# Giovannibriglia/ContinuousBayesianNetwork

Hardware: AMD Instinct MI355X
Metric: marginal queries/sec + achieved HBM GB/s, 20-node d=32 DAG, 65k-batch VE (higher is better)
Workload: dtype f32; 1 GPU; chain20_d32: BayesianNetwork.infer target X19, evidence on the other 19 nodes, N_max=32; queries_per_gpu=65536, global_batch=65536, parallelism=query-shard x1

## Files before the change

continuousbayesiannetwork_amd/csrc/cbn_infer.hip:

```cpp

#include <hip/hip_runtime.h>

#include <algorithm>
#include <cstdarg>
#include <cstdint>
#include <cstdio>
#include <cstdlib>
#include <cstring>
#include <string>
#include <type_traits>
#include <vector>

#include <unistd.h>

#include "cbn_internal.h"

using namespace cbn;

namespace {
thread_local std::string g_err;
}

namespace {
const bool g_diag = [] {
// ... 109 lines not shown
__device__ unsigned g_clock_n = 0;
#define CBN_STAMP_INIT                                                                        \
    const unsigned long long _t0 = __builtin_amdgcn_s_memrealtime();                          \
    const unsigned long long _m0 = __builtin_amdgcn_s_memtime();                              \
    (void)_m0;                                                                                \
    unsigned long long* const _stp = g_stamps;                                                \
    if (_stp && (threadIdx.x & 63) == 0)                                                      \
        _stp[((size_t)blockIdx.x * (blockDim.x / 64) + threadIdx.x / 64) * 12] = _t0
#define CBN_STAMP(k)                                                                          \
    do {                                                                                      \
        __builtin_amdgcn_sched_barrier(0);                                                    \
        unsigned long long _t = __builtin_amdgcn_s_memrealtime();    \
        if (_stp && (threadIdx.x & 63) == 0)                                                  \
            _stp[((size_t)blockIdx.x * (blockDim.x / 64) + threadIdx.x / 64) * 12 + (k)] = _t; \
        __builtin_amdgcn_sched_barrier(0);                                                    \
    } while (0)
#define CBN_CLOCK_END                                                                         \
    do {                                                                                      \
        unsigned long long* const _ck = g_clock;                                              \
        if (_ck && blockIdx.x == 0 && threadIdx.x == 0) {                                     \
            const unsigned long long _m1 = __builtin_amdgcn_s_memtime();                      \
            const unsigned long long _r1 = __builtin_amdgcn_s_memrealtime();                  \
            const unsigned _i = g_clock_n;                                                    \
            if (_i < kClockRing) {                                                            \
                _ck[4 * _i] = _m0;                                                            \
                _ck[4 * _i + 1] = _t0;                                                        \
                _ck[4 * _i + 2] = _m1;                                                        \
                _ck[4 * _i + 3] = _r1;                                                        \
            }                                                                                 \
            g_clock_n = _i + 1;                                                               \
        }                                                                                     \
    } while (0)
#else
#define CBN_STAMP_INIT do {} while (0)
#define CBN_STAMP(k) do {} while (0)
#define CBN_CLOCK_END do {} while (0)
#endif

#ifdef CBN_CHECKED
__device__ unsigned* g_dbg = nullptr;
#define CBN_OK_OR(cond, code) ((cond) ? true : (g_dbg ? (atomicOr(g_dbg, 1u << (code)), atomicAdd(g_dbg + 1 + (code), 1u), false) : false))
#else
#define CBN_OK_OR(cond, code) true
#endif

typedef __attribute__((address_space(3))) void lds_void_t;
typedef const __attribute__((address_space(1))) float gfloat_t;

__device__ __forceinline__ float gload(const float* p, long long i) {
    return ((gfloat_t*)p)[i];
}
typedef const __attribute__((address_space(1))) void gbl_void_t;
typedef const __attribute__((address_space(4))) int cint_t;

typedef unsigned u32x4_t __attribute__((ext_vector_type(4)));
__device__ __forceinline__ __amdgpu_buffer_rsrc_t rows_rsrc(float* base, long long bytes) {
    return __builtin_amdgcn_make_buffer_rsrc(base, 0, (int)(bytes < 0x7fffffff ? bytes : 0x7fffffff), 0x00020000);
}
__device__ __forceinline__ void store_wt(__amdgpu_buffer_rsrc_t r, int off, float4 v) {
    u32x4_t x = {__float_as_uint(v.x), __float_as_uint(v.y), __float_as_uint(v.z), __float_as_uint(v.w)};
#ifndef CBN_STORE_AUX
#define CBN_STORE_AUX 16
#endif
    __builtin_amdgcn_raw_buffer_store_b128(x, r, off, 0, CBN_STORE_AUX);
}

__device__ __forceinline__ int4 sload_int4(const void* p) {
    const cint_t* q = reinterpret_cast<const cint_t*>(reinterpret_cast<uintptr_t>(p));
    return make_int4(q[0], q[1], q[2], q[3]);
}

__device__ __forceinline__ void lds_dma_copy(const float* __restrict__ g, float4* lds, int n4,
                                             int nw = kQueryThreads / kWave) {
    const int lane = threadIdx.x & (kWave - 1);
    const int wave = __builtin_amdgcn_readfirstlane(threadIdx.x / kWave);
    const int nchunk = (n4 + kWave - 1) / kWave;
    for (int c0 = wave; c0 < nchunk; c0 += nw) {
        const int c = (c0 + (int)blockIdx.x) % nchunk;
        const int i = c * kWave + lane;
        if (i < n4 && CBN_OK_OR(i >= 0, 0))
            __builtin_amdgcn_global_load_lds((gbl_void_t*)(g + (size_t)i * 4), (lds_void_t*)(lds + c * kWave), 16,
                                             0, 0);
    }
}

__global__ void k_cpd_scatter(const int32_t* __restrict__ cell, const float* __restrict__ prob,
                              long long n_rows, float* __restrict__ cpd) {
    for (long long r = blockIdx.x * (long long)blockDim.x + threadIdx.x; r < n_rows;
         r += (long long)gridDim.x * blockDim.x)
        cpd[cell[r]] = prob[r];
}

__global__ void k_cpd_normalize(float* __restrict__ cpd, long long n_pcells, int card) {
    for (long long c = blockIdx.x * (long long)blockDim.x + threadIdx.x; c < n_pcells;
         c += (long long)gridDim.x * blockDim.x) {
        float* row = cpd + c * card;
        double s = 0.0;
        for (int v = 0; v < card; ++v) s += (double)row[v];
        const float den = (float)s + 1e-10f;
        for (int v = 0; v < card; ++v) row[v] = row[v] / den;
    }
}

__global__ void k_cpd_eval(const float* __restrict__ cpd, int n_cols, ColPtrs cols,
                           const float* __restrict__ pts, long long n_pts, float* __restrict__ out) {
    for (long long i = blockIdx.x * (long long)blockDim.x + threadIdx.x; i < n_pts;
         i += (long long)gridDim.x * blockDim.x) {
        long long off = 0;
        bool ok = true;
        for (int c = 0; c < n_cols; ++c) {
            const int idx = bsearch_eq(cols.dom[c], cols.card[c], pts[i * n_cols + c]);
            ok &= idx >= 0;
            off += (long long)(idx < 0 ? 0 : idx) * cols.stride[c];
        }
        out[i] = ok ? cpd[off] : 0.f;
    }
}

__device__ double entry_partial(const DevFactor& d, int entry, int N, int c0, int c1, int cs) {
    if (d.kind == CBN_FACTOR_SCALAR) {
        double s = 0.0;
        for (int j = c0; j < c1; j += cs) {
            const int ni = d.node_sample_idx[j];
            s += ni >= 0 ? (double)d.cpd[ni] : 0.0;
        }
        return s;
    }
    const int row = entry / N;
    const int j = entry - row * N;
    const int ni = d.node_sample_idx[j];
    if (ni < 0) return 0.0;
    int base = ni;
    int r = row;
    for (int p = d.n_parents - 1; p >= 0; --p) {
        if (d.ev_slot[p] >= 0) {
            const int card = d.parent_card[p];
            const int q = r / card;
            base += (r - q * card) * d.cpd_stride[p];
            r = q;
        }
    }
    double s = 0.0;
    for (int c = c0; c < c1; c += cs) {
        int off = base;
        int cc = c;
        bool ok = true;
        for (int p = d.n_parents - 1; p >= 0; --p) {
            if (d.ev_slot[p] < 0) {
                const int q = cc / N;
                const int pi = d.parent_sample_idx[p * N + (cc - q * N)];
                cc = q;
                ok &= pi >= 0;
                off += (pi < 0 ? 0 : pi) * d.cpd_stride[p];
            }
        }
        s += ok ? (double)d.cpd[off] : 0.0;
    }
    return s;
}

__device__ __forceinline__ double wave_sum_d(double v) {
#pragma unroll
    for (int o = 32; o > 0; o >>= 1) v += __shfl_xor(v, o, kWave);
    return v;
}

// ... 1157 lines not shown
        }
        if (valid) {
            if (MODE == kModeFused && !first) fq = q;
            if (MODE == kModeWrite) {
                float* o = out + q * N;
#pragma unroll
                for (int v = 0; v < VPL; ++v)
                    *reinterpret_cast<float4*>(o + col[v]) = make_float4(
                        acc[4 * v] / maxv, acc[4 * v + 1] / maxv, acc[4 * v + 2] / maxv, acc[4 * v + 3] / maxv);
            } else if (MODE == kModeRaw) {
                float* o = out + q * N;
#pragma unroll
                for (int v = 0; v < VPL; ++v)
                    *reinterpret_cast<float4*>(o + col[v]) =
                        make_float4(acc[4 * v], acc[4 * v + 1], acc[4 * v + 2], acc[4 * v + 3]);
#pragma unroll
                for (int i = 0; i < NV; ++i) lmax = fmaxf(lmax, acc[i]);
            } else {
#pragma unroll
                for (int i = 0; i < NV; ++i) lmax = fmaxf(lmax, acc[i]);
            }
        }
        __builtin_amdgcn_s_waitcnt(0xC07F);
        __builtin_amdgcn_wave_barrier();
        if (first) CBN_STAMP(6);
        first = false;
    }
    CBN_STAMP(7);
    if (MODE == kModeMax || MODE == kModeRaw) {
        lmax = wave_max(lmax);
        if (lane == 0) wmax[wid] = lmax;
        __syncthreads();
        if (tid == 0) {
            float m = 0.f;
            for (int i = 0; i < nthr / kWave; ++i) m = fmaxf(m, wmax[i]);
            max_out[blockIdx.x] = __float_as_uint(m);
        }
        if (blockIdx.x == 0)
            for (int i = (int)gridDim.x + tid; i < n_max; i += nthr) max_out[i] = 0u;
    }
    if (MODE == kModeFused) {
        lmax = wave_max(lmax);
        if (lane == 0) wmax[wid] = lmax;
        __syncthreads();
        if (wid == 0) {
            const int nw = nthr / kWave;
            const unsigned gm = slot_barrier_max(sync, epoch, wave_max(lane < nw ? wmax[lane] : 0.f));
            if (lane == 0) {
                wmax[0] = __uint_as_float(gm);
                if (blockIdx.x == 0 && max_out) *max_out = gm;
            }
        }
        CBN_STAMP(8);
        __syncthreads();
        CBN_STAMP(9);
        maxv = wmax[0];
        if (fq0 >= 0) {
            float* o = out + fq0 * N;
#pragma unroll
            for (int v = 0; v < VPL; ++v)
                *reinterpret_cast<float4*>(o + col[v]) = make_float4(
                    acc0[4 * v] / maxv, acc0[4 * v + 1] / maxv, acc0[4 * v + 2] / maxv, acc0[4 * v + 3] / maxv);
        }
        if (fq >= 0) {
            float* o = out + fq * N;
#pragma unroll
            for (int v = 0; v < VPL; ++v)
                *reinterpret_cast<float4*>(o + col[v]) = make_float4(
                    acc[4 * v] / maxv, acc[4 * v + 1] / maxv, acc[4 * v + 2] / maxv, acc[4 * v + 3] / maxv);
        }
        CBN_STAMP(10);
    }
}

constexpr int kSR = 256;
constexpr int kSQ = 128;
constexpr int kSU = 4;
#ifndef CBN_DMA_WAVES
#define CBN_DMA_WAVES 4
#endif
constexpr int kDmaW = CBN_DMA_WAVES;
constexpr int kEvW = kQueryThreads / kWave - kDmaW;
constexpr int kSUp = (64 + kEvW - 1) / kEvW;

struct FoldJob {
    float* rows;
    const unsigned* words;
    long long n4;
    long long chunk;
    int n_words;
};
constexpr int kFoldK = 2;
constexpr int kFoldW = 4;

template <int MODE>
__global__ void __launch_bounds__(kQueryThreads)
k_query_staged(const float* __restrict__ gimage, int image_floats, int rec_off, int nf, int zero_off, long long Q,
               long long per, unsigned* __restrict__ sync, unsigned epoch, const unsigned* __restrict__ max_in,
               int n_max, unsigned* __restrict__ max_out, float* __restrict__ out, FoldJob fold,
               FPtrsT<kFastPtrsSmall> fp) {
    CBN_STAMP_INIT;
    constexpr int N = 32;
    extern __shared__ __attribute__((aligned(16))) float4 smem4[];
    float* simg = reinterpret_cast<float*>(smem4);
    const int T = (nf + 2) >> 1;
    const int S = (T + 1) >> 1;
    const int nsl = 4 * (S + 1);
    int* offs = reinterpret_cast<int*>(simg + image_floats);
    float* wmax = reinterpret_cast<float*>(offs + 2 * kSR * nsl);
    const int tid = threadIdx.x;
    const int lane = tid & (kWave - 1);
    const int wid = __builtin_amdgcn_readfirstlane(tid / kWave);
    const long long q0 = (long long)blockIdx.x * per;
    const long long q1 = q0 + per < Q ? q0 + per : Q;
    const int nunits = nf * (kSR / kSQ);
    const FastRec* grec = reinterpret_cast<const FastRec*>(gimage + rec_off);
    const int one_off = zero_off + 64;

    float x[kSUp][2] = {};
    auto stage_load = [&](long long qr, auto ksu, int gw, int GW) {
        constexpr int KSU = decltype(ksu)::value;
        uintptr_t pk[KSU];
#pragma unroll
        for (int k = 0; k < KSU; ++k) {
            const int u = gw + k * GW;
            pk[k] = reinterpret_cast<uintptr_t>(fp.p[((u / (kSR / kSQ)) & 31) * kFastObs]);
        }
#pragma unroll
        for (int k = 0; k < KSU; ++k) {
            const int u = gw + k * GW;
            if (u < nunits) {
                const float* col = reinterpret_cast<const float*>(pk[k] & ~(kTagMore | kTagNone));
#pragma unroll
                for (int h = 0; h < 2; ++h) {
                    const long long q = qr + (u % (kSR / kSQ)) * kSQ + h * kWave + lane;
                    x[k][h] = gload(col, (pk[k] & kTagNone) ? 0 : (q < q1 ? q : q0));
                }
            }
        }
    };
    auto stage_store = [&](long long qr, int buf, auto ksu, int gw, int GW) {
        constexpr int KSU = decltype(ksu)::value;
        int* ob = offs + buf * kSR * nsl;
        int4 rk[KSU];
#pragma unroll
        for (int k = 0; k < KSU; ++k) {
            const int u = gw + k * GW;
            rk[k] = sload_int4(grec + (u < nunits ? u / (kSR / kSQ) : 0));
        }
#pragma unroll
        for (int k = 0; k < KSU; ++k) {
            const int u = gw + k * GW;
            if (u < nunits) {
                const int f = u / (kSR / kSQ);
                const int n_obs = rk[k].y, c0 = rk[k].z;
                const int zoff = zero_off + (f & 1) * 32;
#pragma unroll
                for (int h = 0; h < 2; ++h) {
                    const int ql = (u % (kSR / kSQ)) * kSQ + h * kWave + lane;
                    int o;
                    if (n_obs == 1 && (c0 & kDenseBit)) {
                        const int card = c0 & (kDenseBit - 1);
                        const float xv = x[k][h];
                        const int i = (int)xv;
                        o = (xv >= 0.f && xv < (float)card && (float)i == xv) ? rk[k].x + i * 64 : zoff;
                    } else if (n_obs == 0) {
                        o = rk[k].x;
                    } else {
                        const FastRec& r = grec[f];
                        float xs[kFastObs];
                        xs[0] = x[k][h];
                        if (n_obs > 1) {
                            const long long q = qr + ql;
#pragma unroll
                            for (int p = 1; p < kFastObs; ++p)
                                if (p < n_obs) xs[p] = gload(fp.p[f * kFastObs + p], q < q1 ? q : q0);
                        }
                        int row = 0;
                        bool ok = true;
#pragma unroll
                        for (int p = 0; p < kFastObs; ++p) {
                            if (p < n_obs) {
                                const int card = r.card[p] & (kDenseBit - 1);
                                const float xv = xs[p];
                                int i;
                                if (r.card[p] & kDenseBit) {
                                    i = (int)xv;
                                    i = (xv >= 0.f && xv < (float)card && (float)i == xv) ? i : -1;
                                } else {
                                    i = bsearch_eq(gimage + r.dom_off[p], card, xv);
                                }
                                ok &= i >= 0;
                                row = row * card + (i < 0 ? 0 : i);
                            }
                        }
                        o = ok ? r.table_off + row * 64 : zoff;
                    }
                    ob[ql * nsl + f + ((ql >> 1) & 1)] = o;
                }
            }
        }
    };

    if (tid < kSR) {
        const int d = (tid >> 1) & 1;
        for (int j = 0; j < nsl; ++j) {
            const int f = j - d;
            if (f < 0 || f >= nf) {
                const int o = one_off + (f & 1) * 32;
                offs[tid * nsl + j] = o;
                offs[kSR * nsl + tid * nsl + j] = o;
            }
        }
    }
    long long qr = q0;
    const bool dma_wave = wid < kDmaW;
    if (!dma_wave) {
#ifndef CBN_ABL_NOSTAGE
        if (qr < q1) stage_load(qr, std::integral_constant<int, kSUp>{}, wid - kDmaW, kEvW);
#endif
    } else {
#ifndef CBN_ABL_NODMA
        lds_dma_copy(gimage, smem4, image_floats / 4, kDmaW);
#endif
    }
    CBN_STAMP(1);
    if (!dma_wave && qr < q1)
        stage_store(qr, 0, std::integral_constant<int, kSUp>{}, wid - kDmaW, kEvW);
    CBN_STAMP(2);
    __syncthreads();
    CBN_STAMP(3);
    float4 fv[kFoldK];
    unsigned fw[kFoldW];
    const long long fb = (long long)blockIdx.x * fold.chunk;
    const long long fe = fb + fold.chunk < fold.n4 ? fb + fold.chunk : fold.n4;
    if (MODE == kModeRaw && fold.rows) {
        const float4* r4 = reinterpret_cast<const float4*>(fold.rows);
#pragma unroll
        for (int k = 0; k < kFoldK; ++k) {
            const long long i = fb + tid + k * kQueryThreads;
            fv[k] = i < fe ? r4[i] : make_float4(0.f, 0.f, 0.f, 0.f);
        }
#pragma unroll
        for (int k = 0; k < kFoldW; ++k) {
            const int w = lane + k * kWave;
            fw[k] = w < fold.n_words ? fold.words[w] : 0u;
        }
    }

    const int qi = lane >> 2;
    const int l = lane & 3;
    const int h0 = qi & 1;
    const int clo = (l + 4 * h0) * 4, chi = (l + 4 * (h0 ^ 1)) * 4;
    float lmax = 0.f;
    float maxv = 1.f;
    if (MODE == kModeWrite) {
        unsigned m = 0;
        for (int i = lane; i < n_max; i += kWave) m = max(m, max_in[i]);
        m = wave_max_u(m);
        maxv = __uint_as_float(m);
        if (max_out && blockIdx.x == 0 && tid == 0) *max_out = m;
    }
    float acc[8];
    long long fq = -1;
    int buf = 0;
    const bool wt_raw = MODE == kModeRaw && fold.rows != nullptr;
    const __amdgpu_buffer_rsrc_t orsrc =
        rows_rsrc((MODE == kModeFused || wt_raw) ? out + q0 * N : nullptr,
                  (MODE == kModeFused || wt_raw) ? (q1 - q0) * (long long)(N * 4) : 0);
    for (; qr < q1; qr += kSR, buf ^= 1) {
        const long long qn = qr + kSR;
        if (MODE != kModeFused && qn < q1) stage_load(qn, std::integral_constant<int, kSU>{}, wid, kQueryThreads / kWave);
        const int ql = wid * 16 + qi;
        const long long q = qr + ql;
        const int* my = offs + buf * kSR * nsl + ql * nsl;
#pragma unroll
        for (int i = 0; i < 8; ++i) acc[i] = 1.f;
        auto mul_step = [&](const float4& r0, const float4& r1, const float4& r2, const float4& r3) {
            acc[0] *= r0.x; acc[1] *= r0.y; acc[2] *= r0.z; acc[3] *= r0.w;
            acc[4] *= r1.x; acc[5] *= r1.y; acc[6] *= r1.z; acc[7] *= r1.w;
            acc[0] *= r2.x; acc[1] *= r2.y; acc[2] *= r2.z; acc[3] *= r2.w;
            acc[4] *= r3.x; acc[5] *= r3.y; acc[6] *= r3.z; acc[7] *= r3.w;
        };
        auto load_step = [&](int oa, int ob, float4& r0, float4& r1, float4& r2, float4& r3) {
            r0 = *reinterpret_cast<const float4*>(simg + oa + clo);
            r1 = *reinterpret_cast<const float4*>(simg + oa + chi);
            r2 = *reinterpret_cast<const float4*>(simg + ob + clo);
            r3 = *reinterpret_cast<const float4*>(simg + ob + chi);
        };
        typedef float vf4 __attribute__((ext_vector_type(4)));
        typedef const volatile __attribute__((address_space(3))) vf4 lds_vf4;
        auto vld = [&](int o) {
            const vf4 v = *(lds_vf4*)(simg + o);
            return make_float4(v.x, v.y, v.z, v.w);
        };
        auto vload_step = [&](int oa, int ob, float4& r0, float4& r1, float4& r2, float4& r3) {
            r0 = vld(oa + clo);
            r1 = vld(oa + chi);
            r2 = vld(ob + clo);
            r3 = vld(ob + chi);
        };
        float4 A0, A1, A2, A3, B0, B1, B2, B3;
        int4 on = *reinterpret_cast<const int4*>(my);
        vload_step(on.x, on.y, A0, A1, A2, A3);
        vload_step(on.z, on.w, B0, B1, B2, B3);
        {
            typedef int vi4 __attribute__((ext_vector_type(4)));
            typedef const volatile __attribute__((address_space(3))) vi4 lds_vi4;
            const vi4 v = *(lds_vi4*)(my + 4);
            on = make_int4(v.x, v.y, v.z, v.w);
        }
        CBN_STAMP(4);
#ifdef CBN_ABL_NOPROD
        mul_step(A0, A1, A2, A3);
#else
#pragma unroll 2
        for (int sp = 0; sp < S; ++sp) {
            mul_step(A0, A1, A2, A3);
            load_step(on.x, on.y, A0, A1, A2, A3);
            mul_step(B0, B1, B2, B3);
            load_step(on.z, on.w, B0, B1, B2, B3);
            on = *reinterpret_cast<const int4*>(my + 4 * min(sp + 2, S));
        }
#endif
        CBN_STAMP(5);
        if (q < q1) {
            if (MODE == kModeFused) fq = q;
            if (MODE == kModeRaw && wt_raw) {
                const int ob = (int)(q - q0) * (N * 4);
                store_wt(orsrc, ob + clo * 4, make_float4(acc[0], acc[1], acc[2], acc[3]));
                store_wt(orsrc, ob + chi * 4, make_float4(acc[4], acc[5], acc[6], acc[7]));
            } else if (MODE == kModeWrite || MODE == kModeRaw) {
                const float dv = MODE == kModeWrite ? maxv : 1.f;
                float* o = out + q * N;
                *reinterpret_cast<float4*>(o + clo) = MODE == kModeWrite
                    ? make_float4(acc[0] / dv, acc[1] / dv, acc[2] / dv, acc[3] / dv)
                    : make_float4(acc[0], acc[1], acc[2], acc[3]);
                *reinterpret_cast<float4*>(o + chi) = MODE == kModeWrite
                    ? make_float4(acc[4] / dv, acc[5] / dv, acc[6] / dv, acc[7] / dv)
                    : make_float4(acc[4], acc[5], acc[6], acc[7]);
            }
            if (MODE != kModeWrite)
#pragma unroll
                for (int i = 0; i < 8; ++i) lmax = fmaxf(lmax, acc[i]);
        }
        if (MODE != kModeFused && qn < q1) {
            stage_store(qn, buf ^ 1, std::integral_constant<int, kSU>{}, wid, kQueryThreads / kWave);
            __syncthreads();
        }
    }
    CBN_STAMP(6);
    if (MODE == kModeRaw && fold.rows) {
        unsigned m = 0;
#pragma unroll
        for (int k = 0; k < kFoldW; ++k) m = max(m, fw[k]);
        m = wave_max_u(m);
        const double y = 1.0 / (double)__uint_as_float(m);
        float4* r4 = reinterpret_cast<float4*>(fold.rows);
        const __amdgpu_buffer_rsrc_t frsrc = rows_rsrc(fold.rows + fb * 4, fe > fb ? (fe - fb) * 16 : 0);
#pragma unroll
        for (int k = 0; k < kFoldK; ++k) {
            const long long i = fb + tid + k * kQueryThreads;
            if (i < fe)
                store_wt(frsrc, (int)(i - fb) * 16,
                         make_float4((float)((double)fv[k].x * y), (float)((double)fv[k].y * y),
                                     (float)((double)fv[k].z * y), (float)((double)fv[k].w * y)));
        }
        for (long long i = fb + tid + kFoldK * kQueryThreads; i < fe; i += kQueryThreads) {
            const float4 v = r4[i];
            r4[i] = make_float4((float)((double)v.x * y), (float)((double)v.y * y), (float)((double)v.z * y),
                                (float)((double)v.w * y));
        }
    }
    if (MODE == kModeMax || MODE == kModeRaw) {
        lmax = wave_max(lmax);
        if (lane == 0) wmax[wid] = lmax;
        __syncthreads();
        if (tid == 0) {
            float m = 0.f;
            for (int i = 0; i < kQueryThreads / kWave; ++i) m = fmaxf(m, wmax[i]);
            max_out[blockIdx.x] = __float_as_uint(m);
        }
        if (blockIdx.x == 0)
            for (int i = (int)gridDim.x + tid; i < n_max; i += kQueryThreads) max_out[i] = 0u;
    }
    if (MODE == kModeFused) {
        lmax = wave_max(lmax);
        if (lane == 0) wmax[wid] = lmax;
        __syncthreads();
        CBN_STAMP(7);
        if (wid == 0) {
#ifdef CBN_ABL_NOBAR
            const unsigned gm = __float_as_uint(wave_max(lane < kQueryThreads / kWave ? wmax[lane] : 0.f));
#else
            const unsigned gm = slot_barrier_max(sync, epoch, wave_max(lane < kQueryThreads / kWave ? wmax[lane] : 0.f));
#endif
            if (lane == 0) {
                wmax[0] = __uint_as_float(gm);
                if (blockIdx.x == 0 && max_out) *max_out = gm;
            }
        }
        CBN_STAMP(8);
        __syncthreads();
        CBN_STAMP(9);
        maxv = wmax[0];
// ... 100 lines not shown

int cbn::num_cu() {
    if (g_num_cu == 0) {
        int dev = 0;
        if (hipGetDevice(&dev) != hipSuccess) return 256;
        hipDeviceProp_t prop;
        if (hipGetDeviceProperties(&prop, dev) != hipSuccess) return 256;
        g_num_cu = prop.multiProcessorCount > 0 ? prop.multiProcessorCount : 256;
    }
    return g_num_cu;
}

int cbn::launch_scale(float* out, long long n, const unsigned* words, int n_words, unsigned* pub, hipStream_t s) {
    static const int per_cu = [] {
        const char* e = diag_env("CBN_SCALE_CAP");
        const int x = e ? atoi(e) : 0;
        return x >= 1 && x <= 32 ? x : 4;
    }();
    long long blocks = (n / 4 + 255) / 256;
    const long long cap = (long long)per_cu * num_cu();
    if (blocks > cap) blocks = cap;
    if (blocks < 1) blocks = 1;
    hipLaunchKernelGGL(k_scale, dim3((unsigned)blocks), dim3(256), 0, s, out, n, words, n_words, pub);
    HIP_TRY(hipGetLastError());
    return CBN_OK;
}

namespace {

template <int NP>
FPtrsT<NP> fast_ptrs(const cbn_plan* p, const EvPtrs& ev, int first_factor = 0) {
    FPtrsT<NP> fp;
    const float* dummy = p->ns > 0 ? ev.p[0] : p->d_image;
    for (int i = 0; i < NP; ++i) {
        const int j = i + first_factor * kFastObs;
        fp.p[i] = j < kFastPtrs && p->fast_slot[j] >= 0 ? ev.p[p->fast_slot[j]] : nullptr;
    }
    for (int f = 0; f < NP / kFastObs; ++f) {
        uintptr_t v = reinterpret_cast<uintptr_t>(fp.p[f * kFastObs]);
        if (!v) v = reinterpret_cast<uintptr_t>(dummy) | kTagNone;
        if (fp.p[f * kFastObs + 1]) v |= kTagMore;
        fp.p[f * kFastObs] = reinterpret_cast<const float*>(v);
    }
    return fp;
}

FPtrsT<kFastPtrsSmall> slot_ptrs(const cbn_plan* p, const EvPtrs& ev) {
    FPtrsT<kFastPtrsSmall> sp;
    for (int i = 0; i < kFastPtrsSmall; ++i) sp.p[i] = i < p->ns ? ev.p[i] : nullptr;
    return sp;
}

size_t slots_lds_bytes(long long lds_tab_floats, int ns, int nf, int QB) {
    const size_t nf4 = (size_t)((nf + 3) & ~3);
    const size_t SQ = (size_t)slots_sidx_stride(kQueryThreads / QB);
    size_t b = (size_t)lds_tab_floats * 4 + (size_t)ns * sizeof(QSlot) + (size_t)nf * sizeof(ColRec) +
               (size_t)((ns + 1) & ~1) * sizeof(void*) + ((((size_t)ns * SQ + 7) & ~size_t(7)) * 2) +
               (size_t)QB * nf4 * 4 + (kQueryThreads / kWave) * 4 + 64;
    return (b + 15) & ~size_t(15);
}

template <int VPL, bool LDS, int MODE, int NP>
void launch_fast_np(const cbn_plan* p, unsigned blocks, hipStream_t s, const EvPtrs& ev, long long Q, int L,
                    unsigned epoch, const unsigned* max_in, int n_max, unsigned* max_out, float* out) {
    hipLaunchKernelGGL((k_query_fast<VPL, LDS, MODE, NP>), dim3(blocks), dim3(kQueryThreads), p->fast_lds_bytes, s,
                       p->rec_off, p->nf, p->ns, p->d_image, p->image_floats, fast_ptrs<NP>(p, ev), Q,
                       (Q + blocks - 1) / blocks, p->N, p->RS, L, p->paired ? 1 : 0, p->d_sync, epoch, max_in, n_max,
                       max_out, out, p->lds_tab_floats, p->lds_tab_mask[0], p->lds_tab_mask[1]);
}

template <int VPL, bool LDS, int MODE>
void launch_fast_k(const cbn_plan* p, unsigned blocks, hipStream_t s, const EvPtrs& ev, long long Q, int L,
                   unsigned epoch, const unsigned* max_in, int n_max, unsigned* max_out, float* out,
                   const FoldJob* fold = nullptr) {
    if (p->staged) {
        FoldJob fj;
        memset(&fj, 0, sizeof(fj));
        if (fold && fold->rows && fold->n4 > 0) {
            fj = *fold;
            fj.chunk = (fj.n4 + blocks - 1) / blocks;
        }
        hipLaunchKernelGGL((k_query_staged<MODE>), dim3(blocks), dim3(kQueryThreads), p->staged_lds_bytes, s,
                           p->d_image, p->image_floats, p->rec_off + p->prefix * kRecFloats, p->nf - p->prefix,
                           p->zero_off, Q, (Q + blocks - 1) / blocks, p->d_sync, epoch, max_in, n_max, max_out, out,
                           fj, fast_ptrs<kFastPtrsSmall>(p, ev, p->prefix));
        return;
    }
    if (p->slots) {
        const int QBs = kQueryThreads / L;
        long long per = (Q + blocks - 1) / blocks;
        int coal = per > 2LL * QBs && !diag_env("CBN_SLOTS_NO_COAL") ? 1 : 0;
        if (diag_env("CBN_SLOTS_COAL")) coal = 1;
        for (int i = 0; i < p->ns; ++i) coal &= (reinterpret_cast<uintptr_t>(ev.p[i]) & 15) == 0 ? 1 : 0;
        if (coal) per = (per + 3) & ~3LL;
        hipLaunchKernelGGL((k_query_slots<VPL, MODE>), dim3(blocks), dim3(kQueryThreads), p->fast_lds_bytes, s, p->nf,
                           p->ns, p->d_image, p->rec_off + p->nf * kRecFloats, p->d_crec, slot_ptrs(p, ev), Q, per,
                           p->N, L, p->d_sync, epoch, max_in, n_max, max_out, out, p->lds_tab_floats,
                           p->lds_tab_mask[0], p->lds_tab_mask[1], coal);
        return;
    }
    if (p->cols) {
        auto k = (p->ns + L - 1) / L <= 16 ? k_query_cols<VPL, LDS, MODE, 16> : k_query_cols<VPL, LDS, MODE, 40>;
        hipLaunchKernelGGL(k, dim3(blocks), dim3(kQueryThreads), p->fast_lds_bytes, s,
                           p->rec_off, p->nf, p->ns, p->d_image, p->image_floats, slot_ptrs(p, ev), Q,
                           (Q + blocks - 1) / blocks, p->N, p->RS, L, p->d_sync, epoch, max_in, n_max, max_out, out,
                           p->lds_tab_floats, p->d_crec);
        return;
    }
    if (p->nf * kFastObs <= kFastPtrsSmall)
        launch_fast_np<VPL, LDS, MODE, kFastPtrsSmall>(p, blocks, s, ev, Q, L, epoch, max_in, n_max, max_out, out);
    else
        launch_fast_np<VPL, LDS, MODE, kFastPtrs>(p, blocks, s, ev, Q, L, epoch, max_in, n_max, max_out, out);
}

template <int VPL, bool LDS, int MODE>
const void* fast_kernel_fn(int nf, bool cols = false, int slots_per_lane = 0) {
    if (cols)
        return slots_per_lane <= 16 ? reinterpret_cast<const void*>(&k_query_cols<VPL, LDS, MODE, 16>)
                                    : reinterpret_cast<const void*>(&k_query_cols<VPL, LDS, MODE, 40>);
    return nf * kFastObs <= kFastPtrsSmall ? reinterpret_cast<const void*>(&k_query_fast<VPL, LDS, MODE, kFastPtrsSmall>)
                                           : reinterpret_cast<const void*>(&k_query_fast<VPL, LDS, MODE, kFastPtrs>);
}

template <int VPL, bool LDS, int MODE>
void allow_fast_lds(int bytes) {
    (void)hipFuncSetAttribute(reinterpret_cast<const void*>(&k_query_slots<VPL, MODE>),
                              hipFuncAttributeMaxDynamicSharedMemorySize, bytes);
    (void)hipFuncSetAttribute(reinterpret_cast<const void*>(&k_query_fast<VPL, LDS, MODE, kFastPtrsSmall>),
                              hipFuncAttributeMaxDynamicSharedMemorySize, bytes);
    (void)hipFuncSetAttribute(reinterpret_cast<const void*>(&k_query_fast<VPL, LDS, MODE, kFastPtrs>),
                              hipFuncAttributeMaxDynamicSharedMemorySize, bytes);
    (void)hipFuncSetAttribute(reinterpret_cast<const void*>(&k_query_cols<VPL, LDS, MODE, 16>),
                              hipFuncAttributeMaxDynamicSharedMemorySize, bytes);
    (void)hipFuncSetAttribute(reinterpret_cast<const void*>(&k_query_cols<VPL, LDS, MODE, 40>),
                              hipFuncAttributeMaxDynamicSharedMemorySize, bytes);
}

template <int VPL, bool LDS, bool WRITE>
int launch_fast_v(cbn_plan* p, long long Q, const EvPtrs& ev, const unsigned* max_in, int n_max, unsigned* max_out,
                  float* out, hipStream_t s) {
    const int L = p->N / (4 * VPL);
    const long long cap = p->max_slots;
    long long blocks = (Q * L + kQueryThreads - 1) / kQueryThreads;
    if (blocks > cap) blocks = cap;
    if (!WRITE) n_max = p->max_slots;
    launch_fast_k<VPL, LDS, WRITE ? kModeWrite : kModeMax>(p, (unsigned)blocks, s, ev, Q, L, 0u, max_in, n_max,
                                                          max_out, out);
    HIP_TRY(hipGetLastError());
    return CBN_OK;
}

template <int VPL, bool LDS>
int launch_fused_v(cbn_plan* p, long long Q, const EvPtrs& ev, unsigned* max_bits, float* out, hipStream_t s) {
    const int L = p->N / (4 * VPL);
    const long long per_block = (long long)(kQueryThreads / kWave) * (kWave / L);
    long long blocks = (Q + per_block - 1) / per_block;
    if ((p->slots || p->cols) && CBN_SLOTS_FUSED2) blocks = std::min<long long>(blocks, std::min<long long>(num_cu(), kMaxSlots));
    const unsigned epoch = ++p->fused_epoch;
    if (p->fused_epoch == 0xFFFFFFFFu) p->fused_epoch = 0;
    launch_fast_k<VPL, LDS, kModeFused>(p, (unsigned)blocks, s, ev, Q, L, epoch, nullptr, 0, max_bits, out);
    HIP_TRY(hipGetLastError());
    return CBN_OK;
}

int raw_reserve_cu() {
    static int v = [] {
        const char* e = diag_env("CBN_RAW_RESERVE_CU");
// ... 405 lines not shown
    P->build_units = units;

    bool ok = hipMalloc(&P->d_fac, sizeof(DevFactor) * n_factors) == hipSuccess &&
              hipMalloc(&P->d_slots, sizeof(QSlot) * std::max(ns, 1)) == hipSuccess &&
              hipMalloc(&P->d_build, sizeof(BuildItem) * std::max<size_t>(build.size(), 1)) == hipSuccess &&
              hipMalloc(&P->d_image, sizeof(float) * std::max<long long>(off, 4)) == hipSuccess &&
              hipMalloc(&P->d_sync, sizeof(unsigned) * kSyncWords) == hipSuccess;
    ok = ok && hipMemcpy(P->d_fac, fac.data(), sizeof(DevFactor) * n_factors, hipMemcpyHostToDevice) == hipSuccess;
    ok = ok && (ns == 0 || hipMemcpy(P->d_slots, qs.data(), sizeof(QSlot) * ns, hipMemcpyHostToDevice) == hipSuccess);
    ok = ok && (build.empty() ||
                hipMemcpy(P->d_build, build.data(), sizeof(BuildItem) * build.size(), hipMemcpyHostToDevice) == hipSuccess);
    ok = ok && hipMemset(P->d_image, 0, sizeof(float) * std::max<long long>(off, 4)) == hipSuccess;
    if (ok && paired) {
        const std::vector<float> ones(64, 1.f);
        ok = hipMemcpy(P->d_image + zero_off + 64, ones.data(), sizeof(float) * 64, hipMemcpyHostToDevice) == hipSuccess;
    }
    ok = ok && hipMemset(P->d_sync, 0, sizeof(unsigned) * kSyncWords) == hipSuccess;
    ok = ok && hipHostMalloc(reinterpret_cast<void**>(&P->h_status), sizeof(unsigned),
                             hipHostMallocMapped | hipHostMallocCoherent) == hipSuccess;
    if (ok) {
        *P->h_status = 0;
        unsigned* dh = nullptr;
        ok = hipHostGetDevicePointer(reinterpret_cast<void**>(&dh), P->h_status, 0) == hipSuccess &&
             hipMemcpy(P->d_sync + kHostStatusWordOff, &dh, sizeof(dh), hipMemcpyHostToDevice) == hipSuccess;
    }
    for (int sl = 0; ok && sl < ns; ++sl)
        ok = hipMemcpy(P->d_image + qs[sl].dom_off, slot_dom[sl], sizeof(float) * slot_card[sl],
                       hipMemcpyDeviceToDevice) == hipSuccess;
    ok = ok && hipDeviceSynchronize() == hipSuccess;
    if (!ok) {
        cbn_plan_destroy(P);
        return set_err(CBN_E_HIP, "cbn_plan_create: device allocation/upload failed");
    }

    bool fast = vec == 4 && n_factors * kFastObs <= kFastPtrs;
    std::vector<FastRec> recs(n_factors);
    for (int& sl : P->fast_slot) sl = -1;
    for (int f = 0; f < n_factors && fast; ++f) {
        FastRec& r = recs[f];
        memset(&r, 0, sizeof(r));
        r.table_off = fac[f].table_off;
        for (int p = 0; p < fac[f].n_parents; ++p) {
            const int sl = fac[f].ev_slot[p];
            if (sl >= 0) {
                if (r.n_obs == kFastObs) { fast = false; break; }
                r.card[r.n_obs] = fac[f].parent_card[p] | (qs[sl].dense ? kDenseBit : 0);
                r.dom_off[r.n_obs] = qs[sl].dom_off;
                r.slot[r.n_obs] = sl;
                P->fast_slot[f * kFastObs + r.n_obs] = sl;
                ++r.n_obs;
            }
        }
    }
    int vpl = 0, Lf = 0;
    if (fast) {
        int want = 2;
        if (const char* e = diag_env("CBN_FAST_VPL")) want = atoi(e);
        for (int c : {2, 1}) {
            if (c > want || (N / 4) % c) continue;
            const int Lc = N / (4 * c);
            if (Lc <= kWave && (kWave % Lc) == 0) { vpl = c; Lf = Lc; break; }
        }
        fast = vpl > 0;
    }
    if (fast) {
        const int nf4 = (n_factors + 3) & ~3;
        const size_t side = (size_t)kFastPtrs * sizeof(void*) +
                            (size_t)(kQueryThreads / kWave) * (kWave / Lf) * nf4 * 4 + (kQueryThreads / kWave) * 4 + 64;
        const bool lds_ok = img_bytes + side <= (size_t)kLdsBudget;
        if (!lds_ok && P->use_lds) fast = false;
        if (!P->use_lds && (size_t)P->lds_tab_floats * 4 + (size_t)n_factors * kRecFloats * 4 + side > (size_t)kLdsBudget)
            fast = false;
        if (fast) {
            P->fast = true;
            P->vpl = vpl;
            P->paired = paired && vpl == 2 && P->use_lds;
            const int st_T = (n_factors - P->prefix + 2) >> 1, st_S = (st_T + 1) >> 1;
            const size_t st_bytes =
                img_bytes + (size_t)2 * kSR * (4 * (st_S + 1)) * 4 + (kQueryThreads / kWave) * 4 + 64;
            if (P->paired && (n_factors - P->prefix) * kFastObs <= kFastPtrsSmall && st_bytes <= (size_t)kLdsBudget &&
                !diag_env("CBN_NO_STAGED")) {
                P->staged = true;
                P->staged_lds_bytes = (st_bytes + 15) & ~size_t(15);
                for (const void* fn : {reinterpret_cast<const void*>(&k_query_staged<kModeMax>),
                                       reinterpret_cast<const void*>(&k_query_staged<kModeWrite>),
                                       reinterpret_cast<const void*>(&k_query_staged<kModeFused>),
                                       reinterpret_cast<const void*>(&k_query_staged<kModeRaw>)})
                    (void)hipFuncSetAttribute(fn, hipFuncAttributeMaxDynamicSharedMemorySize, kLdsBudget);
            }
            P->fast_lds_bytes =
                ((P->use_lds ? img_bytes : (size_t)P->lds_tab_floats * 4 + (size_t)n_factors * kRecFloats * 4) + side +
                 15) & ~size_t(15);
            if (!P->staged && !P->paired && Lf <= 2 && ns <= kFastPtrsSmall && n_factors <= kWave &&
                !diag_env("CBN_NO_COLS")) {
                bool ok_c = true;
                for (int sl = 0; sl < ns; ++sl) ok_c = ok_c && slot_card[sl] <= 32767;
                for (int f = 0; f < n_factors && ok_c; ++f)
                    for (int q = 0; q < recs[f].n_obs; ++q)
                        ok_c = ok_c && (recs[f].card[q] & (kDenseBit - 1)) == slot_card[recs[f].slot[q]];
                const size_t QBc = (size_t)kQueryThreads / Lf;
                const size_t cols_bytes =
                    ((P->use_lds ? img_bytes
                                 : (size_t)P->lds_tab_floats * 4 + ((size_t)n_factors * kRecFloats + (size_t)ns * 4) * 4) +
                     (size_t)((ns + 1) & ~1) * sizeof(void*) + (((size_t)ns * QBc + 1) & ~size_t(1)) * 2 +
                     (kQueryThreads / kWave) * 4 + 64 + 16 + (size_t)N * 4 + 15) & ~size_t(15);
                std::vector<ColRec> cr(n_factors);
                for (int f = 0; f < n_factors && ok_c; ++f) {
                    ColRec& c = cr[f];
                    memset(&c, 0, sizeof(c));
                    c.base = recs[f].table_off;
                    c.n_obs = recs[f].n_obs;
                    c.lds = P->use_lds || ((lds_mask[f >> 6] >> (f & 63)) & 1ull) ? 1 : 0;
                    long long w = RS;
                    for (int q = recs[f].n_obs - 1; q >= 0; --q) {
                        ok_c = ok_c && w < (1LL << 24) && recs[f].slot[q] < 256;
                        c.par[q] = (recs[f].slot[q] << 24) | (int)(w & 0xFFFFFF);
                        w *= recs[f].card[q] & (kDenseBit - 1);
                    }
                }
                if (ok_c && cols_bytes <= (size_t)kLdsBudget) {
                    ok_c = hipMalloc(&P->d_crec, sizeof(ColRec) * n_factors) == hipSuccess &&
                           hipMemcpy(P->d_crec, cr.data(), sizeof(ColRec) * n_factors, hipMemcpyHostToDevice) ==
                               hipSuccess;
                    if (!ok_c) {
                        cbn_plan_destroy(P);
                        return set_err(CBN_E_HIP, "cbn_plan_create: column records upload failed");
                    }
                    P->cols = true;
                    P->fast_lds_bytes = cols_bytes;
                }
            }
            if (!P->staged && !P->paired && !P->cols && !P->use_lds && Lf > 2 && ns <= kFastPtrsSmall &&
                n_factors <= 128 && !diag_env("CBN_NO_SLOTS")) {
                bool ok_s = true;
                for (int sl = 0; sl < ns; ++sl) ok_s = ok_s && slot_card[sl] <= 32767;
                for (int f = 0; f < n_factors && ok_s; ++f)
                    for (int q = 0; q < recs[f].n_obs; ++q)
                        ok_s = ok_s && (recs[f].card[q] & (kDenseBit - 1)) == slot_card[recs[f].slot[q]];
                std::vector<ColRec> cr(n_factors);
                for (int f = 0; f < n_factors && ok_s; ++f) {
                    ColRec& c = cr[f];
                    memset(&c, 0, sizeof(c));
                    c.base = recs[f].table_off;
                    c.n_obs = recs[f].n_obs;
                    c.lds = ((lds_mask[f >> 6] >> (f & 63)) & 1ull) ? 1 : 0;
                    long long w = RS;
                    for (int q = recs[f].n_obs - 1; q >= 0; --q) {
                        ok_s = ok_s && w < (1LL << 24) && recs[f].slot[q] < 256;
                        c.par[q] = (recs[f].slot[q] << 24) | (int)(w & 0xFFFFFF);
                        w *= recs[f].card[q] & (kDenseBit - 1);
                    }
                    ok_s = ok_s && (long long)recs[f].table_off + w < (1LL << 31);
                }
                const size_t sb = slots_lds_bytes(P->lds_tab_floats, ns, n_factors, kQueryThreads / Lf);
                if (ok_s && sb <= (size_t)kLdsBudget) {
                    if (hipMalloc(&P->d_crec, sizeof(ColRec) * n_factors) != hipSuccess ||
                        hipMemcpy(P->d_crec, cr.data(), sizeof(ColRec) * n_factors, hipMemcpyHostToDevice) !=
                            hipSuccess) {
                        cbn_plan_destroy(P);
                        return set_err(CBN_E_HIP, "cbn_plan_create: slot records upload failed");
                    }
                    P->slots = true;
                    P->fast_lds_bytes = sb;
                }
            }
            P->fast_blocks_per_cu = 2 * P->fast_lds_bytes <= (size_t)kLdsBudget ? 2 : 1;
// ... 414 lines not shown
```

continuousbayesiannetwork_amd/csrc/cbn_internal.h:

```cpp
#ifndef CBN_INTERNAL_H
#define CBN_INTERNAL_H

#include <hip/hip_runtime.h>

#include <cstdint>

#include "../../include/cbn_amd.h"

namespace cbn {

constexpr int kWave = 64;
constexpr int kLdsBudget = 160 * 1024;
constexpr int kFastPtrs = 416;

constexpr int kSyncLine = 32;
constexpr int kHostStatusWordOff = 8;
constexpr int kMaxSlots = 1024;
constexpr int kSlotWordOff = kSyncLine;
constexpr int kMaxWordOff = kSlotWordOff + 2 * kMaxSlots;
constexpr int kSyncWords = kMaxWordOff + kMaxSlots;

struct DevFactor;
struct QSlot;
struct BuildItem;
struct ParamPlan;
struct DirectPlan;

int set_err(int code, const char* fmt, ...);
const char* diag_env(const char* name);
int num_cu();

int launch_scale(float* out, long long n, const unsigned* words, int n_words, unsigned* pub, hipStream_t s);

int param_run(cbn_plan* plan, int64_t n_queries, const float* const* evidence, int32_t n_evidence,
              uint32_t* max_bits, float* out, int32_t flags, hipStream_t s);
void param_destroy(ParamPlan* pp);
int param_max_words(const ParamPlan* pp);

int direct_run(cbn_plan* plan, int64_t n_queries, const float* const* evidence, int32_t n_evidence,
               uint32_t* max_bits, float* out, int32_t flags, hipStream_t s);
int direct_build_consts(DirectPlan* dp, hipStream_t s);
void direct_destroy(DirectPlan* dp);
int direct_max_words(const DirectPlan* dp);

}

struct cbn_plan {
    int nf = 0;
    int ns = 0;
    int N = 0;
    int vec = 1;
    int L = 1;
    int CH = 1;
    cbn::DevFactor* d_fac = nullptr;
    int* d_crec = nullptr;
    cbn::QSlot* d_slots = nullptr;
    cbn::BuildItem* d_build = nullptr;
    int n_build = 0;
    int build_units = 0;
    float* d_image = nullptr;
    unsigned* d_sync = nullptr;
    bool fast = false;
    int fast_slot[cbn::kFastPtrs];
    static constexpr int kRing = 512;
    hipEvent_t ev[kRing][3] = {};
    int ev_n = 0;
    int rec_off = 0;
    int RS = 1;
    int vpl = 1;
    bool paired = false;
    bool staged = false;
    size_t staged_lds_bytes = 0;
    bool cols = false;
    bool slots = false;
    int zero_off = -1;
    int prefix = 0;
    int prefix_offs[9] = {};
    int prefix_rows = 0;
    unsigned* h_status = nullptr;
    unsigned fused_epoch = 0;
    bool fused_ok = false;
    size_t fast_lds_bytes = 0;
    int lds_tab_floats = 0;
    unsigned long long lds_tab_mask[2] = {0, 0};
    int fast_blocks_per_cu = 1;
    int max_slots = 0;
    int image_floats = 0;
    int table_floats = 0;
    bool use_lds = false;
    size_t lds_bytes = 0;
    int blocks_per_cu = 1;
    cbn::ParamPlan* param = nullptr;
    cbn::DirectPlan* direct = nullptr;
};

#endif
```

Baseline: 6.490 billion queries/s.

## Split LDS image fill so early factor pairs overlap the remaining DMA

Adds an optional split fill of the LDS image using raw global_load_lds asm. Blocks wait only for the chunks the first factor pairs need, start the product loop, then wait for the remaining chunks at a seam barrier. The host computes how many factor pairs fit in the first chunk range. By default the fill is limited to the image prefix up to zero_off, and pad-slot setup moves to evaluation waves. The split path is off unless CBN_FILL_B is set, and the raw waitcnt/barrier code risks ordering bugs.

```diff
diff --git a/continuousbayesiannetwork_amd/csrc/cbn_infer.hip b/continuousbayesiannetwork_amd/csrc/cbn_infer.hip
--- a/continuousbayesiannetwork_amd/csrc/cbn_infer.hip
+++ b/continuousbayesiannetwork_amd/csrc/cbn_infer.hip
@@ -215,6 +215,24 @@
             __builtin_amdgcn_global_load_lds((gbl_void_t*)(g + (size_t)i * 4), (lds_void_t*)(lds + c * kWave), 16,
                                              0, 0);
     }
+}
+
+#pragma clang diagnostic push
+#pragma clang diagnostic ignored "-Winline-asm"
+__device__ __forceinline__ void lds_dma_chunk_asm(const float* g, unsigned lds_addr) {
+    asm volatile("s_mov_b32 m0, %1\n\ts_nop 0\n\tglobal_load_lds_dwordx4 %0, off" ::"v"(g), "s"(lds_addr)
+                 : "memory", "m0");
+}
+#pragma clang diagnostic pop
+template <int K>
+__device__ __forceinline__ void lds_dma_wait() {
+    static_assert(K >= 0 && K < 64, "vmcnt is a 6-bit counter");
+    asm volatile("s_waitcnt vmcnt(%0)" ::"n"(K) : "memory");
+}
+__device__ __forceinline__ void lds_barrier_raw() {
+    asm volatile("s_waitcnt lgkmcnt(0)" ::: "memory");
+    __builtin_amdgcn_s_barrier();
+    asm volatile("" ::: "memory");
 }
 
 __global__ void k_cpd_scatter(const int32_t* __restrict__ cell, const float* __restrict__ prob,
@@ -1538,6 +1556,10 @@
 constexpr int kDmaW = CBN_DMA_WAVES;
 constexpr int kEvW = kQueryThreads / kWave - kDmaW;
 constexpr int kSUp = (64 + kEvW - 1) / kEvW;
+#ifndef CBN_FILL_B
+#define CBN_FILL_B 0
+#endif
+constexpr int kFillB = CBN_FILL_B;
 
 struct FoldJob {
     float* rows;
@@ -1552,9 +1574,9 @@
 template <int MODE>
 __global__ void __launch_bounds__(kQueryThreads)
 k_query_staged(const float* __restrict__ gimage, int image_floats, int rec_off, int nf, int zero_off, long long Q,
-               long long per, unsigned* __restrict__ sync, unsigned epoch, const unsigned* __restrict__ max_in,
-               int n_max, unsigned* __restrict__ max_out, float* __restrict__ out, FoldJob fold,
-               FPtrsT<kFastPtrsSmall> fp) {
+               long long per, unsigned* __restrict__ sync, unsigned epoch, int split,
+               const unsigned* __restrict__ max_in, int n_max, unsigned* __restrict__ max_out,
+               float* __restrict__ out, FoldJob fold, FPtrsT<kFastPtrsSmall> fp) {
     CBN_STAMP_INIT;
     constexpr int N = 32;
     extern __shared__ __attribute__((aligned(16))) float4 smem4[];
@@ -1658,33 +1680,67 @@
         }
     };
 
-    if (tid < kSR) {
-        const int d = (tid >> 1) & 1;
+    auto pad_slots = [&](int t) {
+        const int d = (t >> 1) & 1;
         for (int j = 0; j < nsl; ++j) {
             const int f = j - d;
             if (f < 0 || f >= nf) {
                 const int o = one_off + (f & 1) * 32;
-                offs[tid * nsl + j] = o;
-                offs[kSR * nsl + tid * nsl + j] = o;
-            }
-        }
-    }
+                offs[t * nsl + j] = o;
+                if (MODE != kModeFused) offs[kSR * nsl + t * nsl + j] = o;
+            }
+        }
+    };
     long long qr = q0;
     const bool dma_wave = wid < kDmaW;
+    const int fill_n4 = (zero_off + 128) / 4;
+    const int n_a = split & 0xffff;
+    const int spl = kFillB > 0 ? split >> 16 : 0;
     if (!dma_wave) {
 #ifndef CBN_ABL_NOSTAGE
         if (qr < q1) stage_load(qr, std::integral_constant<int, kSUp>{}, wid - kDmaW, kEvW);
 #endif
+        for (int t = tid - kDmaW * kWave; t < kSR; t += kEvW * kWave) pad_slots(t);
     } else {
 #ifndef CBN_ABL_NODMA
-        lds_dma_copy(gimage, smem4, image_floats / 4, kDmaW);
+        if (kFillB > 0) {
+            const unsigned lds0 =
+                __builtin_amdgcn_readfirstlane((unsigned)reinterpret_cast<uintptr_t>((lds_void_t*)smem4));
+            const int zc0 = spl > 0 ? zero_off / 256 : 0;
+            const int ca = n_a + (fill_n4 + kWave - 1) / kWave - zc0;
+            int a = (wid + (int)blockIdx.x) % ca;
+            for (int a0 = wid; a0 < ca; a0 += kDmaW) {
+                const int c = a < n_a ? a : a - n_a + zc0;
+                const int i = c * kWave + lane;
+                if (i < fill_n4) lds_dma_chunk_asm(gimage + (size_t)i * 4, lds0 + c * 1024);
+                a += kDmaW;
+                while (a >= ca) a -= ca;
+            }
+            if (spl > 0) {
+#pragma unroll
+                for (int k = 0; k < kFillB; ++k) {
+                    const int c = n_a + (wid + k * kDmaW + (int)blockIdx.x) % (kDmaW * kFillB);
+                    lds_dma_chunk_asm(gimage + (size_t)(c * kWave + lane) * 4, lds0 + c * 1024);
+                }
+            }
+        } else {
+            lds_dma_copy(gimage, smem4, fill_n4, kDmaW);
+        }
 #endif
     }
     CBN_STAMP(1);
     if (!dma_wave && qr < q1)
         stage_store(qr, 0, std::integral_constant<int, kSUp>{}, wid - kDmaW, kEvW);
     CBN_STAMP(2);
-    __syncthreads();
+    if (kFillB > 0) {
+        if (dma_wave) {
+            if (spl > 0 && qr < q1) lds_dma_wait<kFillB>();
+            else lds_dma_wait<0>();
+        }
+        lds_barrier_raw();
+    } else {
+        __syncthreads();
+    }
     CBN_STAMP(3);
     float4 fv[kFoldK];
     unsigned fw[kFoldW];
@@ -1758,25 +1814,46 @@
         };
         float4 A0, A1, A2, A3, B0, B1, B2, B3;
         int4 on = *reinterpret_cast<const int4*>(my);
-        vload_step(on.x, on.y, A0, A1, A2, A3);
-        vload_step(on.z, on.w, B0, B1, B2, B3);
-        {
+        auto prime = [&](int sp0) {
+            vload_step(on.x, on.y, A0, A1, A2, A3);
+            vload_step(on.z, on.w, B0, B1, B2, B3);
             typedef int vi4 __attribute__((ext_vector_type(4)));
             typedef const volatile __attribute__((address_space(3))) vi4 lds_vi4;
-            const vi4 v = *(lds_vi4*)(my + 4);
+            const vi4 v = *(lds_vi4*)(my + 4 * min(sp0 + 1, S));
             on = make_int4(v.x, v.y, v.z, v.w);
-        }
+        };
+        auto pairs = [&](int lo, int hi) {
+#pragma unroll 2
+            for (int sp = lo; sp < hi; ++sp) {
+                mul_step(A0, A1, A2, A3);
+                load_step(on.x, on.y, A0, A1, A2, A3);
+                mul_step(B0, B1, B2, B3);
+                load_step(on.z, on.w, B0, B1, B2, B3);
+                on = *reinterpret_cast<const int4*>(my + 4 * min(sp + 2, S));
+            }
+        };
+        const bool seam = kFillB > 0 && spl > 0 && qr == q0;
+        prime(0);
         CBN_STAMP(4);
 #ifdef CBN_ABL_NOPROD
         mul_step(A0, A1, A2, A3);
+        if (seam) {
+            if (dma_wave) lds_dma_wait<0>();
+            lds_barrier_raw();
+            CBN_STAMP(11);
+        }
 #else
-#pragma unroll 2
-        for (int sp = 0; sp < S; ++sp) {
+        if (!seam) {
+            pairs(0, S);
+        } else {
+            pairs(0, spl - 1);
             mul_step(A0, A1, A2, A3);
-            load_step(on.x, on.y, A0, A1, A2, A3);
             mul_step(B0, B1, B2, B3);
-            load_step(on.z, on.w, B0, B1, B2, B3);
-            on = *reinterpret_cast<const int4*>(my + 4 * min(sp + 2, S));
+            if (dma_wave) lds_dma_wait<0>();
+            lds_barrier_raw();
+            CBN_STAMP(11);
+            prime(spl);
+            pairs(spl, S);
         }
 #endif
         CBN_STAMP(5);
@@ -2043,7 +2120,8 @@
         }
         hipLaunchKernelGGL((k_query_staged<MODE>), dim3(blocks), dim3(kQueryThreads), p->staged_lds_bytes, s,
                            p->d_image, p->image_floats, p->rec_off + p->prefix * kRecFloats, p->nf - p->prefix,
-                           p->zero_off, Q, (Q + blocks - 1) / blocks, p->d_sync, epoch, max_in, n_max, max_out, out,
+                           p->zero_off, Q, (Q + blocks - 1) / blocks, p->d_sync, epoch,
+                           fj.rows ? 0 : p->split_chunks | (p->split_pairs << 16), max_in, n_max, max_out, out,
                            fj, fast_ptrs<kFastPtrsSmall>(p, ev, p->prefix));
         return;
     }
@@ -2615,6 +2693,23 @@
                 !diag_env("CBN_NO_STAGED")) {
                 P->staged = true;
                 P->staged_lds_bytes = (st_bytes + 15) & ~size_t(15);
+                const long long zc0 = zero_off / 256, nA = zc0 - (long long)kDmaW * kFillB;
+                if (kFillB > 0 && nA >= 1 && nA < (1 << 15)) {
+                    const int nfs = n_factors - P->prefix;
+                    int sp = 0;
+                    for (; sp < st_S; ++sp) {
+                        bool in_a = true;
+                        for (int f = std::max(4 * sp - 1, 0); f <= 4 * sp + 3 && f < nfs; ++f) {
+                            const DevFactor& d = fac[P->prefix + f];
+                            in_a = in_a && (d.table_off & ~63) + (long long)d.rows * 64 <= nA * 256;
+                        }
+                        if (!in_a) break;
+                    }
+                    if (sp > 0 && sp < st_S) {
+                        P->split_chunks = (int)nA;
+                        P->split_pairs = sp;
+                    }
+                }
                 for (const void* fn : {reinterpret_cast<const void*>(&k_query_staged<kModeMax>),
                                        reinterpret_cast<const void*>(&k_query_staged<kModeWrite>),
                                        reinterpret_cast<const void*>(&k_query_staged<kModeFused>),
diff --git a/continuousbayesiannetwork_amd/csrc/cbn_internal.h b/continuousbayesiannetwork_amd/csrc/cbn_internal.h
--- a/continuousbayesiannetwork_amd/csrc/cbn_internal.h
+++ b/continuousbayesiannetwork_amd/csrc/cbn_internal.h
@@ -71,6 +71,8 @@
     bool paired = false;
     bool staged = false;
     size_t staged_lds_bytes = 0;
+    int split_chunks = 0;
+    int split_pairs = 0;
     bool cols = false;
     bool slots = false;
     int zero_off = -1;
```

New measurement: 6.374 billion queries/s. 0.982x the previous value.
